# linyicheng1/trackingBench-SLAM

Measured on AMD Instinct MI355X. Metric: frames/sec end-to-end (extract+match+local-BA), higher is better.
Workload: dtype u8 (pyramid/FAST/ORB/Hamming) + f64 (pose-opt/BA); 1 GPU; 1280x720 stereo, 8-level pyramid x0.8, 2000 kpts/image (FAST 80/30), searchByBF L<->R, pose-opt, 10-KF/5000-pt local BA x10 iters; distinct_synthetic_pairs=64, distinct_ba_windows=32, ba_partitions=3, ba_schedule=joined at the end of every step, parallelism=frames sharded x1, RCCL gather of tracks

## Files before the change

trackingbench_slam_amd/csrc/k_describe.hip:

```cpp
#include "tb_internal.h"
#include "tb_device.h"

struct DsPattern { float v[1024]; };
constexpr DsPattern ds_make_pattern() {
    constexpr int8_t raw[1024] = {
#include "orb_pattern.inc"
    };
    DsPattern p{};
    for (int i = 0; i < 1024; i++) p.v[i] = (float)raw[i];
    return p;
}
__constant__ __attribute__((aligned(16))) DsPattern c_patternf = ds_make_pattern();

struct DsDisc { uint32_t w1[16][8], wu[16][8]; };
constexpr DsDisc ds_make_disc() {
    constexpr int umax[16] = {15, 15, 15, 15, 14, 14, 14, 13, 13, 12, 11, 10, 9, 8, 6, 3};
    DsDisc d{};
    for (int av = 0; av < 16; av++)
        for (int i = 0; i < 32; i++) {
            const int u = i - 15;
            const bool in = (u >= -umax[av]) && (u <= umax[av]);
            d.w1[av][i >> 2] |= (uint32_t)(in ? 1 : 0) << (8 * (i & 3));
            d.wu[av][i >> 2] |= (uint32_t)(in ? (u + 16) : 0) << (8 * (i & 3));
        }
    return d;
}
__constant__ __attribute__((aligned(16))) DsDisc c_disc = ds_make_disc();

#define DS_P 45
#define DS_PS 84
#define DS_B 39
#define DS_HS 42
#define DS_BS 40

typedef unsigned short ds_u16x2 __attribute__((ext_vector_type(2)));

__device__ __forceinline__ int ds_reflect(int i, int n) {
    if (i < 0) i = -i;
    if (i >= n) i = 2 * (n - 1) - i;
    return i;
}

__device__ __forceinline__ uint32_t ds_window(const uint32_t* w, int o) {
    return (o & 3) ? __builtin_amdgcn_alignbyte(w[(o >> 2) + 1], w[o >> 2], o & 3) : w[o >> 2];
}

__device__ __forceinline__ uint32_t ds_udot2(uint32_t a, uint32_t b, uint32_t c) {
    return __builtin_amdgcn_udot2(__builtin_bit_cast(ds_u16x2, a), __builtin_bit_cast(ds_u16x2, b), c, false);
}

template <int SH>
__device__ __forceinline__ void ds_hrow(const uint32_t* w, unsigned short* out) {
    constexpr uint32_t K1 = 18u | (34u << 8) | (49u << 16) | (55u << 24), K2 = 49u | (34u << 8) | (18u << 16);
    uint32_t a[DS_B + 1];
#pragma unroll
    for (int c = 0; c < DS_B; c++)
        a[c] = __builtin_amdgcn_udot4(ds_window(w, c + SH + 4), K2, __builtin_amdgcn_udot4(ds_window(w, c + SH), K1, 0u, false), false);
    a[DS_B] = 0;
#pragma unroll
    for (int c = 0; c < DS_B; c += 2) *reinterpret_cast<uint32_t*>(out + c) = a[c] | (a[c + 1] << 16);
}

template <int N>
__device__ __forceinline__ void ds_vcol(const uint32_t* h, uint8_t* out) {
    constexpr uint32_t KA = 18u | (34u << 16), KB = 49u | (55u << 16), KC = 49u | (34u << 16);
    uint32_t pr[N + 5];
#pragma unroll
    for (int i = 0; i < N + 5; i++) pr[i] = h[i] | (h[i + 1] << 16);
#pragma unroll
    for (int j = 0; j < N; j++) {
        uint32_t acc = 18u * h[j + 6] + (1u << 15);
        acc = ds_udot2(pr[j], KA, acc);
        acc = ds_udot2(pr[j + 2], KB, acc);
        acc = ds_udot2(pr[j + 4], KC, acc);
        out[j * DS_BS] = (uint8_t)min(acc >> 16, 255u);
    }
}

#define DS_KPB 4

__device__ __forceinline__ void ds_wave_fence() { __builtin_amdgcn_fence(__ATOMIC_SEQ_CST, "workgroup"); }

__global__ void __launch_bounds__(64 * DS_KPB)
k_describe(PlanGeom g, const uint8_t* __restrict__ slab, const uint32_t* __restrict__ sel,
           const int32_t* __restrict__ selCount, tb_keypoint* __restrict__ kps, uint8_t* __restrict__ desc,
           int32_t* __restrict__ counts, int nImages, int by_image, int slotGroups) {
    static_assert(DS_PS == DS_HS * 2, "source rows and h-pass rows share their LDS");
    __shared__ __attribute__((aligned(16))) uint8_t buf_[DS_KPB][DS_P * DS_PS + 16];
    __shared__ int mom[DS_KPB][2];
    __shared__ float rot[DS_KPB][4];
    int b, sg;
    if (by_image) {
        const unsigned L = blockIdx.x, j = L >> 3, grp = j / (unsigned)slotGroups;
        sg = (int)(j - grp * (unsigned)slotGroups);
        b = (int)(grp * 8u + (L & 7u));
        if (b >= nImages) return;
    } else {
        b = blockIdx.y; sg = blockIdx.x;
    }
    const int lane = threadIdx.x & 63;
    const int wave = __builtin_amdgcn_readfirstlane(threadIdx.x >> 6);
    const int slot = sg * DS_KPB + wave;
    uint8_t* const src = buf_[wave];
    unsigned short* const hp = reinterpret_cast<unsigned short*>(buf_[wave]);
    uint8_t* const bl = buf_[wave];
    const int32_t* sc = selCount + b * TB_MAX_LEVELS;
    int level = 0, base = 0;
    for (int l = 0; l < g.nlevels; l++) {
        if (slot >= g.lv[l].selBase) level = l;
    }
    for (int l = 0; l < level; l++) base += sc[l];
    if (slot == 0 && lane == 0) {
        int tot = 0;
        for (int l = 0; l < g.nlevels; l++) tot += sc[l];
        counts[b] = tot;
    }
    const LevelGeom& G = g.lv[level];
    const int idx = slot - G.selBase;
    const bool active = slot < g.selCap && idx < sc[level];
    uint32_t rec = 0;
    int kx = 0, ky = 0, sh = 0;
    if (active) {
        rec = sel[(size_t)b * g.selCap + slot];
        kx = (int)(rec & 0xfff) + TB_BORDER; ky = (int)((rec >> 12) & 0xfff) + TB_BORDER;
        int stride;
        const uint8_t* img = tb_level_ptr(g, slab, b, level, &stride);

        const int x0 = kx - 22, y0 = ky - 22;
        const bool interior = x0 >= 0 && y0 >= 0 && kx + 22 < G.w && ky + 22 < G.h && ((stride & 3) == 0) &&
                              ((reinterpret_cast<uintptr_t>(img) & 3) == 0) && ((x0 & ~3) + 52 <= stride);
        sh = interior ? (x0 & 3) : 0;
        if (interior) {
            const int rr = (lane * 5042) >> 16, dd = lane - rr * 13;
            const uint8_t* srcp = img + (size_t)y0 * stride + (x0 & ~3) + 4 * dd;
            uint32_t v[12];
#pragma unroll
            for (int j = 0; j < 12; j++) {
                const int r = 4 * j + rr;
                v[j] = 0;
                if (rr < 4 && r < DS_P) v[j] = *reinterpret_cast<const uint32_t*>(srcp + (size_t)r * stride);
            }
#pragma unroll
            for (int j = 0; j < 12; j++) {
                const int r = 4 * j + rr;
                if (rr < 4 && r < DS_P) *reinterpret_cast<uint32_t*>(src + r * DS_PS + 4 * dd) = v[j];
            }
        } else {
            for (int e = lane; e < DS_P * DS_P; e += 64) {
                const int r = e / DS_P, c = e - r * DS_P;
                const int yy = ds_reflect(y0 + r, G.h), xx = ds_reflect(x0 + c, G.w);
                src[r * DS_PS + c] = img[(size_t)yy * stride + xx];
            }
        }
        ds_wave_fence();

        int m10 = 0, m01 = 0;
        if (lane < 31) {
            const int v = lane - 15, av = v < 0 ? -v : v;
            const int o = 7 + sh;
            const uint32_t* rw = reinterpret_cast<const uint32_t*>(src + (22 + v) * DS_PS) + (o >> 2);
            const uint4* t1 = reinterpret_cast<const uint4*>(c_disc.w1[av]);
            const uint4* tu = reinterpret_cast<const uint4*>(c_disc.wu[av]);
            const uint4 a0 = t1[0], a1 = t1[1], u0 = tu[0], u1 = tu[1];
            const uint32_t w1[8] = {a0.x, a0.y, a0.z, a0.w, a1.x, a1.y, a1.z, a1.w};
            const uint32_t wu[8] = {u0.x, u0.y, u0.z, u0.w, u1.x, u1.y, u1.z, u1.w};
            uint32_t w[9];
#pragma unroll
            for (int k = 0; k < 9; k++) w[k] = rw[k];
            uint32_t sI = 0, sW = 0;
#pragma unroll
            for (int k = 0; k < 8; k++) {
                const uint32_t X = __builtin_amdgcn_alignbyte(w[k + 1], w[k], (uint32_t)(o & 3));
                sI = __builtin_amdgcn_udot4(X, w1[k], sI, false);
                sW = __builtin_amdgcn_udot4(X, wu[k], sW, false);
            }
            m10 = (int)sW - 16 * (int)sI;
            m01 = v * (int)sI;
        }
        m10 = tb_wave_incl_scan_dpp(m10);
        m01 = tb_wave_incl_scan_dpp(m01);
        if (lane == 63) { mom[wave][0] = m10; mom[wave][1] = m01; }
    }
    __syncthreads();

    if (wave == 0 && lane < DS_KPB) {
        const float angle = tbm::fast_atan2((float)mom[lane][1], (float)mom[lane][0]);
        const float factorPI = (float)(3.1415926535897932384626433832795 / 180.f);
        float a, bsin;
        tbm::sincosf_rn(TB_FMUL(angle, factorPI), &bsin, &a);
        rot[lane][0] = angle; rot[lane][1] = a; rot[lane][2] = bsin;
    }

    if (active) {
        if (lane < DS_P) {
            const uint32_t* rw = reinterpret_cast<const uint32_t*>(src + lane * DS_PS);
            uint32_t w[14];
#pragma unroll
            for (int j = 0; j < 13; j++) w[j] = rw[j];
            w[13] = 0;
            unsigned short* out = hp + lane * DS_HS;
            if (sh == 0) ds_hrow<0>(w, out); else if (sh == 1) ds_hrow<1>(w, out); else if (sh == 2) ds_hrow<2>(w, out); else ds_hrow<3>(w, out);
        }
        ds_wave_fence();
        {
            const int c = lane & 31, r0 = 20 * (lane >> 5);
            const int cc = lane & 7, q0 = 5 * (lane >> 3);
            const int c2 = 32 + min(cc, 6);
            uint32_t h[26], h2[11];
#pragma unroll
            for (int i = 0; i < 26; i++) h[i] = hp[min(r0 + i, DS_P - 1) * DS_HS + c];
#pragma unroll
            for (int i = 0; i < 11; i++) h2[i] = hp[min(q0 + i, DS_P - 1) * DS_HS + c2];
            ds_wave_fence();
            ds_vcol<20>(h, bl + r0 * DS_BS + c);
            ds_vcol<5>(h2, bl + q0 * DS_BS + c2);
        }
    }
    __syncthreads();
    if (!active) return;

    const float angle = rot[wave][0], a = rot[wave][1], bsin = rot[wave][2];
    const uint8_t* center = bl + 19 * DS_BS + 19;
    const size_t out = (size_t)b * g.selCap + base + idx;
    unsigned long long* d64 = reinterpret_cast<unsigned long long*>(desc + out * 32);
    const float4* pat = reinterpret_cast<const float4*>(c_patternf.v);
#pragma unroll
    for (int j = 0; j < 4; j++) {
        const float4 pt = pat[j * 64 + lane];
        const float x0f = pt.x, y0f = pt.y, x1f = pt.z, y1f = pt.w;
        const int r0 = tbm::cv_round(TB_FADD(TB_FMUL(x0f, bsin), TB_FMUL(y0f, a)));
        const int c0 = tbm::cv_round(TB_FSUB(TB_FMUL(x0f, a), TB_FMUL(y0f, bsin)));
        const int r1 = tbm::cv_round(TB_FADD(TB_FMUL(x1f, bsin), TB_FMUL(y1f, a)));
        const int c1 = tbm::cv_round(TB_FSUB(TB_FMUL(x1f, a), TB_FMUL(y1f, bsin)));
        const int t0 = center[r0 * DS_BS + c0], t1 = center[r1 * DS_BS + c1];
        const unsigned long long bits = __ballot(t0 < t1);
        if (lane == 0) d64[j] = bits;
    }

    if (lane == 0) {
        tb_keypoint kp;
        kp.x = (float)kx;
        kp.y = (float)ky;
        if (level != 0) {
            kp.x = TB_FMUL(kp.x, G.sf);
            kp.y = TB_FMUL(kp.y, G.sf);
        }
        kp.size = G.patchSize;
        kp.angle = angle;
        kp.response = (float)(rec >> 24);
        kp.octave = level;
        kp.class_id = -1;
        kps[out] = kp;
    }
}

int tbk_describe(tb_extractor* ex, int n) {
    tb_ctx* ctx = ex->ctx;
    const int by_image = n >= 64 ? 1 : 0;
    const int slotGroups = (ex->g.selCap + DS_KPB - 1) / DS_KPB;
    const dim3 grid = by_image ? dim3((unsigned)slotGroups * 8u * (unsigned)((n + 7) / 8)) : dim3(slotGroups, n);
    tb_prof_begin(ctx, "k_describe");
    hipLaunchKernelGGL(k_describe, grid, dim3(64 * DS_KPB), 0, ctx->stream, ex->g, ex->d_slab, ex->d_sel, ex->d_selCount,
                       ex->d_kps, ex->d_desc, ex->d_counts, n, by_image, slotGroups);
    tb_prof_end(ctx);
    TB_HIP(ctx, hipGetLastError());
    return TB_OK;
}
```

Before: 31760 frames/s.

## Shrink ORB describe patch, transpose h-pass LDS layout, use buffer loads and fast rounding

Cuts the staged patch from 45x45 to 43x43 and brings it in with buffer loads, 9 per lane instead of 12. The horizontal blur pass now writes column-major, so the vertical pass can read packed u16 pairs directly. Both blur passes are grouped into batches of 8 to raise instruction-level parallelism, and all stages share one smaller LDS buffer, which may raise occupancy. Pattern loads are hoisted above the blur, and tap rounding uses a magic-number float trick in place of cv_round. The risk is that the smaller patch margin and the new rounding could change results at patch edges or at exact .5 ties.

Result: faster. 32640 frames/s (median of 6 runs) (+2.8%).

```diff
diff --git a/trackingbench_slam_amd/csrc/k_describe.hip b/trackingbench_slam_amd/csrc/k_describe.hip
--- a/trackingbench_slam_amd/csrc/k_describe.hip
+++ b/trackingbench_slam_amd/csrc/k_describe.hip
@@ -27,11 +27,13 @@
 }
 __constant__ __attribute__((aligned(16))) DsDisc c_disc = ds_make_disc();
 
-#define DS_P 45
-#define DS_PS 84
-#define DS_B 39
-#define DS_HS 42
+#define DS_P 43
+#define DS_PS 52
+#define DS_B 37
+#define DS_CS 46
 #define DS_BS 40
+#define DS_BUF 3408
+static_assert(DS_BUF >= 46 * DS_PS && DS_BUF >= DS_B * DS_CS * 2 && DS_BUF >= 40 * DS_BS && DS_BUF % 16 == 0, "patch buffer tenants");
 
 typedef unsigned short ds_u16x2 __attribute__((ext_vector_type(2)));
 
@@ -49,31 +51,53 @@
     return __builtin_amdgcn_udot2(__builtin_bit_cast(ds_u16x2, a), __builtin_bit_cast(ds_u16x2, b), c, false);
 }
 
+__device__ __forceinline__ int ds_tap(float x, float y, float a, float b) {
+    const float r = TB_FADD(TB_FMUL(x, b), TB_FMUL(y, a)), c = TB_FSUB(TB_FMUL(x, a), TB_FMUL(y, b));
+    constexpr uint32_t M = 0x4B400000u;
+    const uint32_t br = __builtin_bit_cast(uint32_t, TB_FADD(r, 12582912.0f)), bc = __builtin_bit_cast(uint32_t, TB_FADD(c, 12582912.0f));
+    return (int)((uint32_t)__mul24((int)br, DS_BS) + bc - ((M & 0xffffffu) * DS_BS + M));
+}
+
 template <int SH>
 __device__ __forceinline__ void ds_hrow(const uint32_t* w, unsigned short* out) {
     constexpr uint32_t K1 = 18u | (34u << 8) | (49u << 16) | (55u << 24), K2 = 49u | (34u << 8) | (18u << 16);
-    uint32_t a[DS_B + 1];
-#pragma unroll
-    for (int c = 0; c < DS_B; c++)
-        a[c] = __builtin_amdgcn_udot4(ds_window(w, c + SH + 4), K2, __builtin_amdgcn_udot4(ds_window(w, c + SH), K1, 0u, false), false);
-    a[DS_B] = 0;
-#pragma unroll
-    for (int c = 0; c < DS_B; c += 2) *reinterpret_cast<uint32_t*>(out + c) = a[c] | (a[c + 1] << 16);
+    constexpr int GRP = 8;
+#pragma unroll
+    for (int c0 = 0; c0 < DS_B; c0 += GRP) {
+        uint32_t a[GRP];
+#pragma unroll
+        for (int i = 0; i < GRP; i++)
+            if (c0 + i < DS_B) a[i] = __builtin_amdgcn_udot4(ds_window(w, c0 + i + SH), K1, 0u, false);
+#pragma unroll
+        for (int i = 0; i < GRP; i++)
+            if (c0 + i < DS_B) a[i] = __builtin_amdgcn_udot4(ds_window(w, c0 + i + SH + 4), K2, a[i], false);
+#pragma unroll
+        for (int i = 0; i < GRP; i++)
+            if (c0 + i < DS_B) out[(c0 + i) * DS_CS] = (unsigned short)a[i];
+    }
 }
 
 template <int N>
-__device__ __forceinline__ void ds_vcol(const uint32_t* h, uint8_t* out) {
-    constexpr uint32_t KA = 18u | (34u << 16), KB = 49u | (55u << 16), KC = 49u | (34u << 16);
-    uint32_t pr[N + 5];
-#pragma unroll
-    for (int i = 0; i < N + 5; i++) pr[i] = h[i] | (h[i + 1] << 16);
-#pragma unroll
-    for (int j = 0; j < N; j++) {
-        uint32_t acc = 18u * h[j + 6] + (1u << 15);
-        acc = ds_udot2(pr[j], KA, acc);
-        acc = ds_udot2(pr[j + 2], KB, acc);
-        acc = ds_udot2(pr[j + 4], KC, acc);
-        out[j * DS_BS] = (uint8_t)min(acc >> 16, 255u);
+__device__ __forceinline__ void ds_vcol(const uint32_t* P, uint8_t* out) {
+    constexpr uint32_t KE[4] = {18u | (34u << 16), 49u | (55u << 16), 49u | (34u << 16), 18u};
+    constexpr uint32_t KO[4] = {18u << 16, 34u | (49u << 16), 55u | (49u << 16), 34u | (18u << 16)};
+    constexpr int GRP = 8;
+#pragma unroll
+    for (int j0 = 0; j0 < N; j0 += GRP) {
+        uint32_t acc[GRP];
+#pragma unroll
+        for (int k = 0; k < 4; k++)
+#pragma unroll
+            for (int i = 0; i < GRP; i++) {
+                const int j = j0 + i;
+                if (j < N) acc[i] = ds_udot2(P[(j >> 1) + k], (j & 1) ? KO[k] : KE[k], k ? acc[i] : (1u << 15));
+            }
+#pragma unroll
+        for (int i = 0; i < GRP; i++)
+            if (j0 + i < N) acc[i] = min(acc[i] >> 16, 255u);
+#pragma unroll
+        for (int i = 0; i < GRP; i++)
+            if (j0 + i < N) out[(j0 + i) * DS_BS] = (uint8_t)acc[i];
     }
 }
 
@@ -85,8 +109,7 @@
 k_describe(PlanGeom g, const uint8_t* __restrict__ slab, const uint32_t* __restrict__ sel,
            const int32_t* __restrict__ selCount, tb_keypoint* __restrict__ kps, uint8_t* __restrict__ desc,
            int32_t* __restrict__ counts, int nImages, int by_image, int slotGroups) {
-    static_assert(DS_PS == DS_HS * 2, "source rows and h-pass rows share their LDS");
-    __shared__ __attribute__((aligned(16))) uint8_t buf_[DS_KPB][DS_P * DS_PS + 16];
+    __shared__ __attribute__((aligned(16))) uint8_t buf_[DS_KPB][DS_BUF];
     __shared__ int mom[DS_KPB][2];
     __shared__ float rot[DS_KPB][4];
     int b, sg;
@@ -126,25 +149,20 @@
         int stride;
         const uint8_t* img = tb_level_ptr(g, slab, b, level, &stride);
 
-        const int x0 = kx - 22, y0 = ky - 22;
-        const bool interior = x0 >= 0 && y0 >= 0 && kx + 22 < G.w && ky + 22 < G.h && ((stride & 3) == 0) &&
-                              ((reinterpret_cast<uintptr_t>(img) & 3) == 0) && ((x0 & ~3) + 52 <= stride);
+        const int x0 = kx - 21, y0 = ky - 21;
+        const bool interior = x0 >= 0 && y0 >= 0 && kx + 21 < G.w && ky + 21 < G.h && ((stride & 3) == 0) &&
+                              ((reinterpret_cast<uintptr_t>(img) & 3) == 0) && ((x0 & ~3) + 48 <= stride);
         sh = interior ? (x0 & 3) : 0;
         if (interior) {
-            const int rr = (lane * 5042) >> 16, dd = lane - rr * 13;
-            const uint8_t* srcp = img + (size_t)y0 * stride + (x0 & ~3) + 4 * dd;
-            uint32_t v[12];
-#pragma unroll
-            for (int j = 0; j < 12; j++) {
-                const int r = 4 * j + rr;
-                v[j] = 0;
-                if (rr < 4 && r < DS_P) v[j] = *reinterpret_cast<const uint32_t*>(srcp + (size_t)r * stride);
-            }
-#pragma unroll
-            for (int j = 0; j < 12; j++) {
-                const int r = 4 * j + rr;
-                if (rr < 4 && r < DS_P) *reinterpret_cast<uint32_t*>(src + r * DS_PS + 4 * dd) = v[j];
-            }
+            const int rr = (lane * 5462) >> 16, dd = lane - rr * 12;
+            const __amdgpu_buffer_rsrc_t rs = __builtin_amdgcn_make_buffer_rsrc(
+                const_cast<uint8_t*>(img) + (size_t)y0 * stride + (x0 & ~3), 0, (DS_P - 1) * stride + 48, 0x00020000);
+            const int off = rr * stride + 4 * dd;
+            uint32_t v[9];
+#pragma unroll
+            for (int j = 0; j < 9; j++) v[j] = __builtin_amdgcn_raw_buffer_load_b32(rs, off + 5 * j * stride, 0, 0);
+#pragma unroll
+            for (int j = 0; j < 9; j++) *reinterpret_cast<uint32_t*>(src + (5 * j + rr) * DS_PS + 4 * dd) = v[j];
         } else {
             for (int e = lane; e < DS_P * DS_P; e += 64) {
                 const int r = e / DS_P, c = e - r * DS_P;
@@ -157,8 +175,8 @@
         int m10 = 0, m01 = 0;
         if (lane < 31) {
             const int v = lane - 15, av = v < 0 ? -v : v;
-            const int o = 7 + sh;
-            const uint32_t* rw = reinterpret_cast<const uint32_t*>(src + (22 + v) * DS_PS) + (o >> 2);
+            const int o = 6 + sh;
+            const uint32_t* rw = reinterpret_cast<const uint32_t*>(src + (21 + v) * DS_PS) + (o >> 2);
             const uint4* t1 = reinterpret_cast<const uint4*>(c_disc.w1[av]);
             const uint4* tu = reinterpret_cast<const uint4*>(c_disc.wu[av]);
             const uint4 a0 = t1[0], a1 = t1[1], u0 = tu[0], u1 = tu[1];
@@ -191,53 +209,54 @@
         rot[lane][0] = angle; rot[lane][1] = a; rot[lane][2] = bsin;
     }
 
+    float4 pt[4];
+#pragma unroll
+    for (int j = 0; j < 4; j++) pt[j] = reinterpret_cast<const float4*>(c_patternf.v)[j * 64 + lane];
     if (active) {
-        if (lane < DS_P) {
-            const uint32_t* rw = reinterpret_cast<const uint32_t*>(src + lane * DS_PS);
-            uint32_t w[14];
-#pragma unroll
-            for (int j = 0; j < 13; j++) w[j] = rw[j];
-            w[13] = 0;
-            unsigned short* out = hp + lane * DS_HS;
-            if (sh == 0) ds_hrow<0>(w, out); else if (sh == 1) ds_hrow<1>(w, out); else if (sh == 2) ds_hrow<2>(w, out); else ds_hrow<3>(w, out);
+        {
+            const uint32_t* rw = reinterpret_cast<const uint32_t*>(src + min(lane, DS_P - 1) * DS_PS);
+            uint32_t w[12];
+#pragma unroll
+            for (int j = 0; j < 12; j++) w[j] = rw[j];
+            ds_wave_fence();
+            if (lane < DS_P) {
+                unsigned short* out = hp + lane;
+                if (sh == 0) ds_hrow<0>(w, out); else if (sh == 1) ds_hrow<1>(w, out); else if (sh == 2) ds_hrow<2>(w, out); else ds_hrow<3>(w, out);
+            }
         }
         ds_wave_fence();
         {
-            const int c = lane & 31, r0 = 20 * (lane >> 5);
-            const int cc = lane & 7, q0 = 5 * (lane >> 3);
-            const int c2 = 32 + min(cc, 6);
-            uint32_t h[26], h2[11];
-#pragma unroll
-            for (int i = 0; i < 26; i++) h[i] = hp[min(r0 + i, DS_P - 1) * DS_HS + c];
-#pragma unroll
-            for (int i = 0; i < 11; i++) h2[i] = hp[min(q0 + i, DS_P - 1) * DS_HS + c2];
+            const int c = lane & 31, r0 = 18 * (lane >> 5);
+            const int l2 = min(lane, 49), pc = (l2 * 205) >> 10, c2 = 32 + l2 - 5 * pc, q0 = 4 * pc;
+            const uint32_t* p1 = reinterpret_cast<const uint32_t*>(hp + c * DS_CS + r0);
+            const uint32_t* p2 = reinterpret_cast<const uint32_t*>(hp + c2 * DS_CS + q0);
+            uint32_t P[13], P2[5];
+#pragma unroll
+            for (int i = 0; i < 13; i++) P[i] = p1[i];
+#pragma unroll
+            for (int i = 0; i < 5; i++) P2[i] = p2[i];
             ds_wave_fence();
-            ds_vcol<20>(h, bl + r0 * DS_BS + c);
-            ds_vcol<5>(h2, bl + q0 * DS_BS + c2);
+            ds_vcol<19>(P, bl + r0 * DS_BS + c);
+            ds_vcol<4>(P2, bl + q0 * DS_BS + c2);
         }
     }
     __syncthreads();
     if (!active) return;
 
     const float angle = rot[wave][0], a = rot[wave][1], bsin = rot[wave][2];
-    const uint8_t* center = bl + 19 * DS_BS + 19;
+    const uint8_t* center = bl + 18 * DS_BS + 18;
     const size_t out = (size_t)b * g.selCap + base + idx;
     unsigned long long* d64 = reinterpret_cast<unsigned long long*>(desc + out * 32);
-    const float4* pat = reinterpret_cast<const float4*>(c_patternf.v);
+    unsigned long long bits[4];
 #pragma unroll
     for (int j = 0; j < 4; j++) {
-        const float4 pt = pat[j * 64 + lane];
-        const float x0f = pt.x, y0f = pt.y, x1f = pt.z, y1f = pt.w;
-        const int r0 = tbm::cv_round(TB_FADD(TB_FMUL(x0f, bsin), TB_FMUL(y0f, a)));
-        const int c0 = tbm::cv_round(TB_FSUB(TB_FMUL(x0f, a), TB_FMUL(y0f, bsin)));
-        const int r1 = tbm::cv_round(TB_FADD(TB_FMUL(x1f, bsin), TB_FMUL(y1f, a)));
-        const int c1 = tbm::cv_round(TB_FSUB(TB_FMUL(x1f, a), TB_FMUL(y1f, bsin)));
-        const int t0 = center[r0 * DS_BS + c0], t1 = center[r1 * DS_BS + c1];
-        const unsigned long long bits = __ballot(t0 < t1);
-        if (lane == 0) d64[j] = bits;
+        const int t0 = center[ds_tap(pt[j].x, pt[j].y, a, bsin)], t1 = center[ds_tap(pt[j].z, pt[j].w, a, bsin)];
+        bits[j] = __ballot(t0 < t1);
     }
 
     if (lane == 0) {
+#pragma unroll
+        for (int j = 0; j < 4; j++) d64[j] = bits[j];
         tb_keypoint kp;
         kp.x = (float)kx;
         kp.y = (float)ky;
```
